# mcogoni/supersdr

Measured on AMD Instinct MI355X. Metric: real-time IQ channels sustained (WF+demod), higher is better.
Workload: dtype f32

## Files before the change

supersdr_amd/csrc/ssdr_audio_dev.h:

```cpp
#pragma once
#include "ssdr_math.h"
#include "ssdr_kernels.h"

constexpr int OCT = 10;
constexpr int NOCT = (SSDR_HIST + SSDR_FRAME) / 8;
constexpr int HOCT = SSDR_HIST / 8;
typedef uint32_t u32x4 __attribute__((ext_vector_type(4)));

SSDR_DEV void lds_sync()
{
    __builtin_amdgcn_fence(__ATOMIC_RELEASE, "wavefront");
    __builtin_amdgcn_wave_barrier();
    __builtin_amdgcn_fence(__ATOMIC_ACQUIRE, "wavefront");
}

template <int CTRL, int ROWMASK>
SSDR_DEV float dpp(float identity, float x)
{
    return __int_as_float(__builtin_amdgcn_update_dpp(__float_as_int(identity), __float_as_int(x), CTRL, ROWMASK, 0xF, false));
}
SSDR_DEV float vmax(float a, float b)
{
    float r;
    asm("v_max_f32 %0, %1, %2" : "=v"(r) : "v"(a), "v"(b));
    return r;
}
SSDR_DEV float vmax3(float a, float b, float c)
{
    float r;
    asm("v_max3_f32 %0, %1, %2, %3" : "=v"(r) : "v"(a), "v"(b), "v"(c));
    return r;
}
SSDR_DEV float vmax3_abs(float a, float b, float c)
{
    float r;
    asm("v_max3_f32 %0, %1, |%2|, |%3|" : "=v"(r) : "v"(a), "v"(b), "v"(c));
    return r;
}
SSDR_DEV uint32_t lane63_u(uint32_t x) { return (uint32_t)__builtin_amdgcn_readlane((int)x, 63); }
SSDR_DEV uint32_t from_prev_lane_u(uint32_t lane0_value, uint32_t x)
{
    return (uint32_t)__builtin_amdgcn_update_dpp((int)lane0_value, (int)x, 0x138, 0xF, 0xF, false);
}
typedef short s16x2 __attribute__((ext_vector_type(2)));
typedef unsigned short u16x2 __attribute__((ext_vector_type(2)));
SSDR_DEV uint32_t iq_power(uint32_t raw)
{
    uint32_t p;
    asm("v_dot2_i32_i16 %0, %1, %1, 0" : "=v"(p) : "v"(raw));
    return p;
}
SSDR_DEV float lane63(float x) { return __int_as_float(__builtin_amdgcn_readlane(__float_as_int(x), 63)); }
SSDR_DEV float from_prev_lane(float lane0_value, float x) { return dpp<0x138, 0xF>(lane0_value, x); }

#define SSDR_SCAN6(STEP) STEP("row_shr:1", "0xf") STEP("row_shr:2", "0xf") STEP("row_shr:4", "0xf") STEP("row_shr:8", "0xf") \
                         STEP("row_bcast:15", "0xa") STEP("row_bcast:31", "0xc")
#define SSDR_DPP(C, M) " " C " row_mask:" M " bank_mask:0xf"

SSDR_DEV float scan_max(float x)
{
#define STEP(C, M) asm("s_nop 1\n\tv_max_f32_dpp %0, %0, %0" SSDR_DPP(C, M) : "+v"(x));
    SSDR_SCAN6(STEP)
#undef STEP
    return x;
}
SSDR_DEV float scan_sum(float x)
{
#define STEP(C, M) asm("s_nop 1\n\tv_add_f32_dpp %0, %0, %0" SSDR_DPP(C, M) : "+v"(x));
    SSDR_SCAN6(STEP)
#undef STEP
    return x;
}
SSDR_DEV void scan_affine(float &A, float &B)
{
#define STEP(C, M) asm("s_nop 1\n\tv_fmac_f32_dpp %1, %1, %0" SSDR_DPP(C, M) "\n\tv_mul_f32_dpp %0, %0, %0" SSDR_DPP(C, M) : "+v"(A), "+v"(B));
    SSDR_SCAN6(STEP)
#undef STEP
}

struct Nco {
    uint32_t dphi;
    float cs, ss;
    float qc, qs;
    float tc, ts;
};
SSDR_DEV void nco_setup(Nco &n, uint32_t dphi, int l, int block = 8)
{
    n.dphi = dphi;
    ssdr_phasor32(dphi, n.cs, n.ss);
    ssdr_phasor32((uint32_t)(block * l) * dphi, n.qc, n.qs);
    n.tc = 1.0f; n.ts = 0.0f;
}
SSDR_DEV void nco_frame_table(Nco &n, uint32_t phase_of_frame, int l, int frame = SSDR_FRAME)
{
    ssdr_phasor32(phase_of_frame + (uint32_t)(frame * l) * n.dphi, n.tc, n.ts);
}
SSDR_DEV float lane_f(float x, uint32_t lane) { return __int_as_float(__builtin_amdgcn_readlane(__float_as_int(x), (int)lane)); }
SSDR_DEV void nco_block(const Nco &n, uint32_t f, float &c, float &s)
{
    const float fc = lane_f(n.tc, f & 63u), fs = lane_f(n.ts, f & 63u);
    c = fmaf(fc, n.qc, -(fs * n.qs));
    s = fmaf(fs, n.qc, fc * n.qs);
}
SSDR_DEV void phasor_mul(float ac, float as, float bc, float bs, float &c, float &s)
{
    c = fmaf(ac, bc, -(as * bs));
    s = fmaf(as, bc, ac * bs);
}

template <bool CLIP, int N = 8>
SSDR_DEV void mix8(const uint32_t (&rw)[N], float c, float s, float cs, float ss, float2 (&z)[N], float &amax)
{
#pragma unroll
    for (int j = 0; j < N; j++) {
        const float xr = (float)(int16_t)(rw[j] & 0xFFFFu);
        const float xi = (float)((int32_t)rw[j] >> 16);
        if (CLIP) amax = vmax3_abs(amax, xr, xi);
        z[j] = make_float2(fmaf(xr, c, xi * s), fmaf(xi, c, -(xr * s)));
        const float cn = fmaf(c, cs, -(s * ss)), sn = fmaf(s, cs, c * ss);
        c = cn; s = sn;
    }
}

template <bool CLIP>
SSDR_DEV void mix8_carry(const uint32_t *rw, float &c, float &s, float cs, float ss, float2 (&z)[8], float &amax)
{
#pragma unroll
    for (int j = 0; j < 8; j++) {
        const float xr = (float)(int16_t)(rw[j] & 0xFFFFu);
        const float xi = (float)((int32_t)rw[j] >> 16);
        if (CLIP) amax = vmax3_abs(amax, xr, xi);
        z[j] = make_float2(fmaf(xr, c, xi * s), fmaf(xi, c, -(xr * s)));
        const float cn = fmaf(c, cs, -(s * ss)), sn = fmaf(s, cs, c * ss);
        c = cn; s = sn;
    }
}

SSDR_DEV void load_oct(const float2 *z, int q, float2 (&v)[8])
{
    const float4 *p = reinterpret_cast<const float4 *>(z + q * OCT);
#pragma unroll
    for (int i = 0; i < 4; i++) {
        const float4 t = p[i];
        v[2 * i] = make_float2(t.x, t.y);
        v[2 * i + 1] = make_float2(t.z, t.w);
    }
}

SSDR_DEV void store_oct(float2 *z, int q, const float2 (&v)[8])
{
    float4 *p = reinterpret_cast<float4 *>(z + q * OCT);
#pragma unroll
    for (int i = 0; i < 4; i++) p[i] = make_float4(v[2 * i].x, v[2 * i].y, v[2 * i + 1].x, v[2 * i + 1].y);
}

template <int K0, int NK>
SSDR_DEV void fir_taps(const float *h, const float2 (&A)[8], const float2 (&B)[8], float (&yr)[8], float (&yi)[8])
{
#pragma unroll
    for (int kk = K0; kk < K0 + NK; kk++) {
#pragma unroll
        for (int j = 0; j < 8; j++) {
            const float2 v = (j - kk >= 0) ? A[(j - kk) & 7] : B[(8 + j - kk) & 7];
            yr[j] = fmaf(h[kk], v.x, yr[j]);
            yi[j] = fmaf(h[kk], v.y, yi[j]);
        }
    }
}


struct AgcK { float c0, c1, knee, d8; uint32_t K; };

template <bool INTEGER_POWER>
SSDR_DEV void demod_am(const float (&p)[8], float &dc, float (&aud)[8])
{
    constexpr float DC_APOW[8] = SSDR_DC_APOW_INIT;
    float env[8], loc[8];
    float s = 0.0f;
#pragma unroll
    for (int j = 0; j < 8; j++) {
        env[j] = INTEGER_POWER ? ssdr_sqrt_rn_int(p[j]) : ssdr_sqrt_rn(p[j]);
        s = fmaf(SSDR_DC_A, s, SSDR_DC_AL * env[j]);
        loc[j] = s;
    }
    float Asc = DC_APOW[7], Bsc = s;
    scan_affine(Asc, Bsc);
    const float Ae = from_prev_lane(1.0f, Asc), Be = from_prev_lane(0.0f, Bsc);
    const float carry = fmaf(Ae, dc, Be);
    float m = 0.0f;
#pragma unroll
    for (int j = 0; j < 8; j++) {
        m = fmaf(DC_APOW[j], carry, loc[j]);
        aud[j] = env[j] - m;
    }
    dc = lane63(m);
}

SSDR_DEV void demod_ssb(const float (&yr)[8], const float (&yi)[8], float c, float s, float cs2, float ss2, float (&aud)[8])
{
#pragma unroll
    for (int j = 0; j < 8; j++) {
        aud[j] = fmaf(yr[j], c, -(yi[j] * s));
        const float cn = fmaf(c, cs2, -(s * ss2)), sn = fmaf(s, cs2, c * ss2);
        c = cn; s = sn;
    }
}

SSDR_DEV void demod_fm(const float (&yr)[8], const float (&yi)[8], float prev_re, float prev_im, float kfm, float (&aud)[8])
{
    float pr = from_prev_lane(prev_re, yr[7]), pi = from_prev_lane(prev_im, yi[7]);
#pragma unroll
    for (int j = 0; j < 8; j++) {
        const float dr = fmaf(yr[j], pr, yi[j] * pi);
        const float di = fmaf(yi[j], pr, -(yr[j] * pi));
        aud[j] = ssdr_atan2p(di, dr) * kfm;
        pr = yr[j]; pi = yi[j];
    }
}

SSDR_DEV float block_peak(const float (&p)[8])
{
    return vmax3(vmax3(vmax3(p[0], p[1], p[2]), p[3], p[4]), vmax3(p[5], p[6], p[7]), SSDR_P_FLOOR);
}

SSDR_DEV float agc_pack_store(const float (&p)[8], const float (&aud)[8], int l, const AgcK &k, float &agc_d,
                              float (&agc_m)[8], int16_t *dst, float pm_known = -1.0f)
{
    const float pm = pm_known >= 0.0f ? pm_known : block_peak(p);
    const float al = ssdr_log2p(pm);
    const float fl = (float)l;
    const float d8 = k.d8;
    float e;
    if (k.K == 0) {
        const float P = scan_max(fmaf(fl, d8, al));
        e = vmax(fmaf(-fl, d8, P), fmaf(-(fl + 1.0f), d8, agc_d));
        agc_d = lane63(e);
    } else {
        const float P = scan_max(al);
        float maxM = agc_m[0], mK = agc_m[0];
#pragma unroll
        for (int i = 1; i < 8; i++)
            if ((uint32_t)i < k.K) { maxM = fmaxf(maxM, agc_m[i]); mK = agc_m[i]; }
        e = vmax(vmax(P, maxM), fmaf(-(fl + 1.0f), d8, agc_d));
        agc_d = fmaxf(fmaf(-64.0f, d8, agc_d), mK);
#pragma unroll
        for (int i = 7; i > 0; i--) agc_m[i] = agc_m[i - 1];
        agc_m[0] = lane63(P);
    }
    const float g = ssdr_exp2p(fmaf(k.c1, vmax(e, k.knee), k.c0));
    u32x4 w;
#pragma unroll
    for (int j = 0; j < 8; j += 2) {
        const int i0 = __float2int_rn(aud[j] * g), i1 = __float2int_rn(aud[j + 1] * g);
        w[j >> 1] = __builtin_bit_cast(uint32_t, __builtin_amdgcn_cvt_pk_i16(i0, i1));
    }
    SSDR_NT_STORE(w, reinterpret_cast<u32x4 *>(dst));
    return g;
}

template <bool HANG> struct AgcHang { float m[8]; };
template <> struct AgcHang<false> {};

template <bool HANG>
SSDR_DEV void agc_pack_store_fused(const float (&aud)[8], int l, const AgcK &k, float &agc_d, AgcHang<HANG> &hang, int16_t *dst, float pm)
{
    const float al = ssdr_log2p(pm);
    const float fl = (float)l;
    const float d8 = k.d8;
    float e;
    auto no_hang = [&] {
        const float P = scan_max(fmaf(fl, d8, al));
        e = vmax(fmaf(-fl, d8, P), fmaf(-(fl + 1.0f), d8, agc_d));
        agc_d = lane63(e);
    };
    if constexpr (!HANG) {
        no_hang();
    } else if (k.K == 0) {
        no_hang();
    } else {
        float (&agc_m)[8] = hang.m;
        const float P = scan_max(al);
        float maxM = agc_m[0], mK = agc_m[0];
#pragma unroll
        for (int i = 1; i < 8; i++)
            if ((uint32_t)i < k.K) { maxM = fmaxf(maxM, agc_m[i]); mK = agc_m[i]; }
        e = vmax(vmax(P, maxM), fmaf(-(fl + 1.0f), d8, agc_d));
        agc_d = fmaxf(fmaf(-64.0f, d8, agc_d), mK);
#pragma unroll
        for (int i = 7; i > 0; i--) agc_m[i] = agc_m[i - 1];
        agc_m[0] = lane63(P);
    }
    const float g = ssdr_exp2p(fmaf(k.c1, vmax(e, k.knee), k.c0));
    u32x4 w;
#pragma unroll
    for (int j = 0; j < 8; j += 2) {
        const int i0 = __float2int_rn(aud[j] * g), i1 = __float2int_rn(aud[j + 1] * g);
        w[j >> 1] = __builtin_bit_cast(uint32_t, __builtin_amdgcn_cvt_pk_i16(i0, i1));
    }
    SSDR_NT_STORE(w, reinterpret_cast<u32x4 *>(dst));
}

SSDR_DEV void iq_pack_store(const float (&yr)[8], const float (&yi)[8], float g, uint32_t *dst)
{
    u32x4 w0, w1;
#pragma unroll
    for (int j = 0; j < 8; j++) {
        const uint32_t v = __builtin_bit_cast(uint32_t, __builtin_amdgcn_cvt_pk_i16(__float2int_rn(yr[j] * g), __float2int_rn(yi[j] * g)));
        if (j < 4) w0[j] = v; else w1[j - 4] = v;
    }
    SSDR_NT_STORE(w0, reinterpret_cast<u32x4 *>(dst));
    SSDR_NT_STORE(w1, reinterpret_cast<u32x4 *>(dst) + 1);
}

SSDR_DEV void rssi_flag_step(const float (&p)[8], bool clip, uint32_t f, uint32_t n_frames, int l, float cal,
                             float &rssi_sum, uint32_t &flag_keep, float *rssi_row, uint8_t *flag_row)
{
    float ps = p[0];
#pragma unroll
    for (int j = 1; j < 8; j++) ps = ps + p[j];
    const float tot = lane63(scan_sum(ps));
    if ((f & 63u) == (uint32_t)l) { rssi_sum = tot; flag_keep = clip ? 1u : 0u; }
    if ((f & 63u) == 63u || f + 1 == n_frames) {
        if ((uint32_t)l <= (f & 63u)) {
            rssi_row[(f & ~63u) + l] = fmaf(ssdr_log2p(fmaxf(rssi_sum, 1e-20f)) - 39.0f, SSDR_DB_PER_LOG2, cal);
            flag_row[(f & ~63u) + l] = (uint8_t)flag_keep;
        }
    }
}

SSDR_DEV bool wave_any(bool x) { return __builtin_amdgcn_ballot_w64(x) != 0ull; }

SSDR_DEV bool raw_clipped(const uint32_t (&rw)[8])
{
    bool c = false;
#pragma unroll
    for (int j = 0; j < 8; j++) {
        const int lo = (int16_t)(rw[j] & 0xFFFFu), hi = (int32_t)rw[j] >> 16;
        c = c || lo >= 32767 || lo <= -32767 || hi >= 32767 || hi <= -32767;
    }
    return c;
}

SSDR_DEV bool raw_clipped1(uint32_t rw)
{
    const int lo = (int16_t)(rw & 0xFFFFu), hi = (int32_t)rw >> 16;
    return lo >= 32767 || lo <= -32767 || hi >= 32767 || hi <= -32767;
}
SSDR_DEV bool raw_clipped_delayed(const uint32_t (&rw)[8], uint32_t last, int l)
{
    bool head = false, c = raw_clipped1(last);
#pragma unroll
    for (int j = 0; j < 4; j++) head |= raw_clipped1(rw[j]);
#pragma unroll
    for (int j = 4; j < 8; j++) c |= raw_clipped1(rw[j]);
    return c | (head & (l != 0));
}

SSDR_DEV uint32_t scan_add_u(uint32_t x)
{
#define STEP(C, M) asm("s_nop 1\n\tv_add_u32_dpp %0, %0, %0" SSDR_DPP(C, M) : "+v"(x));
    SSDR_SCAN6(STEP)
#undef STEP
    return x;
}
SSDR_DEV uint32_t scan_max_u(uint32_t x)
{
#define STEP(C, M) asm("s_nop 1\n\tv_max_u32_dpp %0, %0, %0" SSDR_DPP(C, M) : "+v"(x));
    SSDR_SCAN6(STEP)
#undef STEP
    return x;
}

struct NbRun { uint32_t gate, thresh, s1, s2, left; };

template <int N>
SSDR_DEV uint32_t nb_frame(uint32_t (&rw)[N], int l, NbRun &s, bool &clip)
{
    constexpr uint32_t M = 64u * N;
    constexpr int SHIFT = __builtin_ctz(M);
    const uint32_t lmin = s.s1 < s.s2 ? s.s1 : s.s2;
    const uint64_t t64 = (uint64_t)s.thresh * lmin;
    const uint32_t tc = (t64 == 0 || t64 >= 0xFFFFFFFFull) ? 0xFFFFFFFFu : (uint32_t)t64;
    uint32_t part = 0, trig = 0;
    u16x2 rails = {0xFFFFu, 0xFFFFu};
#pragma unroll
    for (int j = 0; j < N; j++) {
        const uint32_t p = iq_power(rw[j]);
        part += p >> SHIFT;
        trig |= (uint32_t)(p > tc) << j;
        rails = __builtin_elementwise_min(rails, __builtin_bit_cast(u16x2, rw[j]) + (u16x2){32769u, 32769u});
    }
    clip = wave_any(rails.x < 3u || rails.y < 3u);
    const uint32_t n0 = (uint32_t)(N * l);
    const uint32_t le = trig ? n0 + (31u - (uint32_t)__builtin_clz(trig)) + s.gate : 0u;
    const uint32_t sc = scan_max_u(le);
    const uint32_t from_left = from_prev_lane_u(0u, sc);
    const uint32_t e = s.left > from_left ? s.left : from_left;
    int d = (int)e - (int)n0;
    uint32_t mask = 0;
#pragma unroll
    for (int j = 0; j < N; j++) {
        d = (trig >> j) & 1u ? j + (int)s.gate : d;
        const bool b = j < d;
        mask |= (uint32_t)b << j;
        rw[j] = b ? 0u : rw[j];
    }
    const uint32_t sum = lane63_u(scan_add_u(part));
    const uint32_t last = lane63_u(sc);
    const uint32_t ef = s.left > last ? s.left : last;
    s.left = ef > M ? ef - M : 0u;
    s.s2 = s.s1;
    s.s1 = sum;
    return mask;
}
```

supersdr_amd/csrc/ssdr_wf.hip:

```cpp
#include "ssdr_math.h"
#include "ssdr_kernels.h"
#include "ssdr_audio_dev.h"
#include "ssdr_wf_dev.h"

namespace {

constexpr int WAVES = SSDR_WF_BLOCK / 64;
constexpr int LDS_TOTAL = LDS_XCH + WAVES * 2 * XCH_FLOATS * 4;
static_assert(LDS_TOTAL <= 163840, "LDS budget");

template <bool AVG, bool HOP>
__global__ __launch_bounds__(SSDR_WF_BLOCK, SSDR_WF_WAVES_PER_EU) void ssdr_wf_kernel(SsdrWfArgs a)
{
    __shared__ __attribute__((aligned(16))) unsigned char smem[LDS_TOTAL];
    load_tables(smem, a.win, a.tw_stage, a.lut);

    const int lane = threadIdx.x & 63, wave = __builtin_amdgcn_readfirstlane(threadIdx.x >> 6);
    const int h = lane >> 5, l = lane & 31;
    float *xch_wave = reinterpret_cast<float *>(smem + LDS_XCH) + wave * 2 * XCH_FLOATS;
    const unsigned char *lut = smem + LDS_LUT0;
    const uint32_t n_pairs = (a.n_ch + 1) >> 1;
    const uint32_t run = HOP ? a.grp_run : 1u;
    const uint32_t n_runs = (a.n_groups + run - 1) / run;
    const uint32_t n_items = n_pairs * n_runs;
    const uint32_t wave_stride = gridDim.x * WAVES;

    for (uint32_t item = blockIdx.x * WAVES + wave; item < n_items; item += wave_stride) {
      uint32_t pair, g_begin, g_end;
      if (HOP) {
          pair = item / n_runs;
          g_begin = (item - pair * n_runs) * run;
          g_end = min(g_begin + run, a.n_groups);
      } else {
          g_begin = item / n_pairs;
          pair = item - g_begin * n_pairs;
          g_end = g_begin + 1;
      }
      const uint32_t n_trips = HOP ? g_end - g_begin : 1u;
      for (uint32_t trip = 0; trip < n_trips; trip++) {
        const uint32_t grp = g_begin + trip;
        uint32_t pair_now = __builtin_amdgcn_readfirstlane(pair);
        asm volatile("" : "+s"(pair_now));
        const WfItem it = wf_item(a, pair_now, grp, h);
        const float calq = a.consts[it.ch].wf_cal_lin * SSDR_LUT_SCALE;
        uint32_t acc[AVG ? 16 : 1];
#pragma unroll
        for (int j = 0; j < (AVG ? 16 : 1); j++) acc[j] = 0;
        constexpr uint32_t LINE_STEP = HOP ? SSDR_NFFT / 2 : SSDR_NFFT;
        const uint32_t *src = a.iq + (uint64_t)it.ch * a.ch_stride + (uint64_t)it.l0 * LINE_STEP + l;

        for (uint32_t line = it.l0; line < it.l1; line++, src += LINE_STEP) {
            f32x2 z[32];
            uint32_t raw[32];
            if (HOP) load_line_halves(line ? src - SSDR_NFFT / 2 : a.tail + (uint64_t)it.ch * (SSDR_NFFT / 2) + l, src, raw);
            else load_line(src, raw);
            if (SSDR_PRIO_WF) prio_compute_phase();
            window_line(raw, smem, l, z);
            SCHED_FENCE();
            fft_line<AVG>(z, smem, xch_wave, h, l);
            if (SSDR_PRIO_WF) prio_latency_phase();

            if (AVG) {
                quantise32(z, calq, lut, [&](int j, uint32_t q01) { acc[j] += q01; });
            } else {
                uint32_t q[16];
                quantise32(z, calq, lut, [&](int j, uint32_t q01) { q[j] = q01; });
                int16_t *x16 = reinterpret_cast<int16_t *>(xch_wave + opaque(h) * XCH_FLOATS) + opaque(l);
#pragma unroll
                for (int j = 0; j < 16; j++) {
                    x16[32 * (j + 16)] = (int16_t)(q[j] & 0xFFFFu);
                    x16[32 * j] = (int16_t)(q[j] >> 16);
                }
            }
        }

        float *xch = xch_wave + opaque(h) * XCH_FLOATS;
        if (AVG) {
            int16_t *x16 = reinterpret_cast<int16_t *>(xch) + opaque(l);
#pragma unroll
            for (int j = 0; j < 16; j++) {
                x16[32 * (j + 16)] = (int16_t)(acc[j] & 0xFFFFu);
                x16[32 * j] = (int16_t)(acc[j] >> 16);
            }
        }
        wave_lds_sync();
        const u32x4 *x128 = reinterpret_cast<const u32x4 *>(xch);
        int16_t *dst = it.complete ? a.out + ((uint64_t)it.grp * a.n_ch + it.ch) * SSDR_NFFT
                                   : a.acc_out + (uint64_t)it.ch * SSDR_NFFT;
        const int16_t *cin = a.acc_in + (uint64_t)it.ch * SSDR_NFFT;
#pragma unroll
        for (int q = 0; q < 4; q++) {
            u32x4 v = x128[q * 32 + l];
            if (AVG && it.carry_in)
                v += reinterpret_cast<const u32x4 *>(cin)[q * 32 + l];
            if (it.ch_ok) SSDR_NT_STORE(v, reinterpret_cast<u32x4 *>(dst) + q * 32 + l);
        }
        wave_lds_sync();
      }
    }
}

template <bool HOP, bool AVG = false, bool HANG = true>
__global__ __launch_bounds__(SSDR_WF_BLOCK, SSDR_WF_WAVES_PER_EU) void ssdr_fused_am_kernel(SsdrFusedArgs fa)
{
    __shared__ __attribute__((aligned(16))) unsigned char smem[LDS_TOTAL];
    const SsdrWfArgs &a = fa.wf;
    const SsdrAudioArgs &u = fa.au;
    load_tables(smem, a.win, a.tw_stage, a.lut);

    const int lane = threadIdx.x & 63, wave = __builtin_amdgcn_readfirstlane(threadIdx.x >> 6);
    const int h = lane >> 5, l = lane & 31;
    float *xch_wave = reinterpret_cast<float *>(smem + LDS_XCH) + wave * 2 * XCH_FLOATS;
    uint32_t *qbuf = reinterpret_cast<uint32_t *>(xch_wave);
    const unsigned char *lut = smem + LDS_LUT0;
    const uint32_t n_pairs = (a.n_ch + 1) >> 1;
    const uint32_t wave_stride = gridDim.x * WAVES;
    const uint32_t n_frames = u.n_frames;

    for (uint32_t pair = blockIdx.x * WAVES + wave; pair < n_pairs; pair += wave_stride) {
        const uint32_t ch_raw = 2 * pair + h;
        const bool ch_ok = ch_raw < a.n_ch;
        const uint32_t ch = ch_ok ? ch_raw : a.n_ch - 1;
        const float cal_wf = a.consts[ch].wf_cal_lin * SSDR_LUT_SCALE;
        const uint32_t n_sub = (2 * pair + 1 < a.n_ch) ? 2u : 1u;

        float rssi_sum[2] = {0.0f, 0.0f};
        uint32_t flag_keep[2] = {0u, 0u};
        auto pad = [&](int c, int i) -> float & { return xch_wave[c * XCH_FLOATS + 33 * (i + 17) + 32]; };
        constexpr int PAD_TAIL = HANG ? 10 : 2;
        constexpr bool PARKED = !HOP;
        constexpr int PARK = PARKED ? 4 : 0;
        if (lane < 2) {
            const uint32_t cc = min(2 * pair + (uint32_t)lane, a.n_ch - 1);
            const ssdr_chan_state st = u.state[cc];
            pad(lane, 0) = st.dc;
            pad(lane, 1) = st.agc_d;
            if (HANG) {
#pragma unroll
                for (int i = 0; i < 8; i++) pad(lane, 2 + i) = st.agc_m[i];
            }
            const uint4 t = *reinterpret_cast<const uint4 *>(u.hist + (size_t)cc * SSDR_HIST + SSDR_HIST - 4);
            if constexpr (PARKED) {
                pad(lane, PAD_TAIL) = __uint_as_float(t.x); pad(lane, PAD_TAIL + 1) = __uint_as_float(t.y);
                pad(lane, PAD_TAIL + 2) = __uint_as_float(t.z); pad(lane, PAD_TAIL + 3) = __uint_as_float(t.w);
            } else {
                pad(lane, PAD_TAIL) = __uint_as_float(iq_power(t.x)); pad(lane, PAD_TAIL + 1) = __uint_as_float(iq_power(t.y));
                pad(lane, PAD_TAIL + 2) = __uint_as_float(iq_power(t.z)); pad(lane, PAD_TAIL + 3) = __uint_as_float(iq_power(t.w));
            }
        }
        wave_lds_sync();

        const uint32_t *src = a.iq + (uint64_t)ch * a.ch_stride + l;
        uint32_t last_raw31 = 0;
        uint32_t acc[AVG ? 16 : 1];
#pragma unroll
        for (int j = 0; j < (AVG ? 16 : 1); j++) acc[j] = 0;
        constexpr uint32_t LINE_STEP = HOP ? SSDR_NFFT / 2 : SSDR_NFFT;
        constexpr int FRAMES_PER_LINE = HOP ? 1 : 2;
        for (uint32_t line = 0; line < a.n_lines; line++, src += LINE_STEP) {
            float dc[2], agc_d[2];
            AgcHang<HANG> hang[2];
            uint32_t tail_q[2][4];
#pragma unroll
            for (int c = 0; c < 2; c++) {
                dc[c] = pad(c, 0); agc_d[c] = pad(c, 1);
                if constexpr (HANG) {
#pragma unroll
                    for (int i = 0; i < 8; i++) hang[c].m[i] = pad(c, 2 + i);
                }
                if constexpr (!PARKED) {
#pragma unroll
                    for (int i = 0; i < 4; i++) tail_q[c][i] = __float_as_uint(pad(c, PAD_TAIL + i));
                }
            }
            if constexpr (PARKED) {
                u32x4 b[2];
#pragma unroll
                for (int c = 0; c < 2; c++)
#pragma unroll
                    for (int i = 0; i < 4; i++) b[c][i] = __float_as_uint(pad(c, PAD_TAIL + i));
                wave_lds_sync();
                if (lane == 0) {
#pragma unroll
                    for (int c = 0; c < 2; c++) *reinterpret_cast<u32x4 *>(qbuf + c * XCH_FLOATS) = b[c];
                }
            }
            wave_lds_sync();
            const uint32_t lw = opaque(lane);
            uint32_t *q_park = qbuf + PARK + 4 * lw;
            const uint32_t *q_lane = q_park - PARK + 4 * lw, *q_last = qbuf + (lw & 3u);
            {
                u32x4 t[2][4];
#pragma unroll
                for (int c = 0; c < 2; c++) {
                    uint32_t pair_now = __builtin_amdgcn_readfirstlane(pair);
                    asm volatile("" : "+s"(pair_now));
                    const uint32_t cc = min(2 * pair_now + (uint32_t)c, a.n_ch - 1);
                    const uint32_t *row = a.iq + (uint64_t)cc * a.ch_stride + (uint64_t)line * LINE_STEP;
                    if (HOP) {
                        const uint32_t *older = line ? row - SSDR_NFFT / 2 : a.tail + (uint64_t)cc * (SSDR_NFFT / 2);
#pragma unroll
                        for (int i = 0; i < 2; i++) t[c][i] = SSDR_NT_LOAD(reinterpret_cast<const u32x4 *>(older) + 64 * i + lw);
#pragma unroll
                        for (int i = 0; i < 2; i++) t[c][2 + i] = reinterpret_cast<const u32x4 *>(row)[64 * i + lw];
                    } else {
#pragma unroll
                        for (int i = 0; i < 4; i++) t[c][i] = SSDR_NT_LOAD(reinterpret_cast<const u32x4 *>(row) + 64 * i + lw);
                    }
                }
                SCHED_FENCE();
#pragma unroll
                for (int c = 0; c < 2; c++)
#pragma unroll
                    for (int i = 0; i < 4; i++) reinterpret_cast<u32x4 *>(q_park + c * XCH_FLOATS)[64 * i] = t[c][i];
                SCHED_FENCE();
            }
            wave_lds_sync();
            prio_latency_phase();
#pragma unroll
            for (int c = 0; c < 2; c++) {
                if ((uint32_t)c >= n_sub) continue;
                uint32_t pair_now = __builtin_amdgcn_readfirstlane(pair);
                asm volatile("" : "+s"(pair_now));
                const uint32_t cc = 2 * pair_now + c;
                const ssdr_chan_consts &kc = u.consts[cc];
                const AgcK agc_c = {kc.agc_c0, kc.agc_c1, kc.agc_knee, kc.agc_delta8, kc.hang_frames};
                const float cal_c = kc.smeter_cal_db;
#pragma unroll
                for (int f = 0; f < FRAMES_PER_LINE; f++) {
                    const uint32_t frame = HOP ? line : 2 * line + f;
                    const int FBASE = c * XCH_FLOATS + SSDR_FRAME * (HOP ? 1 : f);
                    const u32x4 *qp = reinterpret_cast<const u32x4 *>(q_lane + FBASE);
                    const u32x4 q0 = qp[0], q1 = qp[1];
                    const uint32_t rw[8] = {q0.x, q0.y, q0.z, q0.w, q1.x, q1.y, q1.z, q1.w};
                    uint32_t d[8];
                    float p[8], aud[8];
                    float pmx;
                    bool trig, clip;
                    if constexpr (PARKED) {
                        const uint32_t last = q_last[FBASE + SSDR_FRAME];
#pragma unroll
                        for (int j = 0; j < 8; j++) d[j] = iq_power(rw[j]);
#pragma unroll
                        for (int j = 0; j < 8; j++) p[j] = (float)d[j];
                        pmx = block_peak(p);
                        trig = wave_any((pmx >= 1073676160.0f) | (iq_power(last) >= 0x3FFF0001u));
                        clip = trig ? wave_any(raw_clipped_delayed(rw, last, lane)) : false;
                    } else {
                        uint32_t qv[8];
#pragma unroll
                        for (int j = 0; j < 8; j++) qv[j] = iq_power(rw[j]);
#pragma unroll
                        for (int j = 0; j < 4; j++) { d[j] = from_prev_lane_u(tail_q[c][j], qv[4 + j]); d[4 + j] = qv[j]; }
#pragma unroll
                        for (int j = 0; j < 4; j++) tail_q[c][j] = lane63_u(qv[4 + j]);
#pragma unroll
                        for (int j = 0; j < 8; j++) p[j] = (float)d[j];
                        pmx = block_peak(p);
                        trig = wave_any(pmx >= 1073676160.0f) || tail_q[c][0] >= 0x3FFF0001u || tail_q[c][1] >= 0x3FFF0001u ||
                               tail_q[c][2] >= 0x3FFF0001u || tail_q[c][3] >= 0x3FFF0001u;
                        clip = trig ? wave_any(raw_clipped(rw)) : false;
                    }
                    demod_am<true>(p, dc[c], aud);
                    agc_pack_store_fused<HANG>(aud, lane, agc_c, agc_d[c], hang[c], u.pcm + ((uint64_t)cc * n_frames + frame) * SSDR_FRAME + 8 * lane, pmx);
                    rssi_flag_step(p, clip, frame, n_frames, lane, cal_c, rssi_sum[c], flag_keep[c],
                                   u.rssi + (uint64_t)cc * n_frames, u.flags + (uint64_t)cc * n_frames);
                }
            }
            wave_lds_sync();
            prio_compute_phase();
            uint32_t raw[32];
            {
                const uint32_t *q = qbuf + opaque(h) * XCH_FLOATS + opaque(l);
#pragma unroll
                for (int r = 0; r < 32; r++) raw[r] = q[PARK + 32 * r];
            }
            wave_lds_sync();
            if (lane < 2) {
#pragma unroll
                for (int c = 0; c < 2; c++) {
                    if (lane != c) continue;
                    pad(c, 0) = dc[c]; pad(c, 1) = agc_d[c];
                    if constexpr (HANG) {
#pragma unroll
                        for (int i = 0; i < 8; i++) pad(c, 2 + i) = hang[c].m[i];
                    }
                    if constexpr (PARKED) {
                        const u32x4 e = *reinterpret_cast<const u32x4 *>(qbuf + c * XCH_FLOATS + PARK + SSDR_NFFT - 4);
#pragma unroll
                        for (int i = 0; i < 4; i++) pad(c, PAD_TAIL + i) = __uint_as_float(e[i]);
                    } else {
#pragma unroll
                        for (int i = 0; i < 4; i++) pad(c, PAD_TAIL + i) = __uint_as_float(tail_q[c][i]);
                    }
                }
            }
            wave_lds_sync();
            SCHED_FENCE();
            if (line + 1 == a.n_lines && ch_ok) {
#pragma unroll
                for (int r = 28; r < 32; r++) u.hist[(size_t)ch * SSDR_HIST + 32 * (r - 28) + l] = raw[r];
            }
            last_raw31 = raw[31];
            uint32_t qn[16];
            f32x2 z[32];
            window_line(raw, smem, l, z);
            SCHED_FENCE();
            fft_line<true>(z, smem, xch_wave, h, l);
            prio_latency_phase();
            if (AVG) quantise32(z, cal_wf, lut, [&](int j, uint32_t q01) { acc[j] += q01; });
            else quantise32(z, cal_wf, lut, [&](int j, uint32_t q01) { qn[j] = q01; });
            const uint32_t pos = a.phase + line;
            const bool group_done = !AVG || (pos + 1) % a.n_avg == 0;
            const bool last_line = line + 1 == a.n_lines;
            if (group_done || last_line) {
                float *xch = xch_wave + opaque(h) * XCH_FLOATS;
                int16_t *x16 = reinterpret_cast<int16_t *>(xch) + opaque(l);
#pragma unroll
                for (int j = 0; j < 16; j++) {
                    const uint32_t v = AVG ? acc[j] : qn[j];
                    x16[32 * (j + 16)] = (int16_t)(v & 0xFFFFu);
                    x16[32 * j] = (int16_t)(v >> 16);
                }
                wave_lds_sync();
                const u32x4 *x128 = reinterpret_cast<const u32x4 *>(xch);
                const uint32_t grp = AVG ? pos / a.n_avg : line;
                int16_t *dst = group_done ? a.out + ((uint64_t)grp * a.n_ch + ch) * SSDR_NFFT : a.acc_out + (uint64_t)ch * SSDR_NFFT;
                const bool carry_in = AVG && grp == 0 && a.phase != 0;
                const int16_t *cin = a.acc_in + (uint64_t)ch * SSDR_NFFT;
#pragma unroll
                for (int q = 0; q < 4; q++) {
                    u32x4 v = x128[q * 32 + l];
                    if (carry_in) v += reinterpret_cast<const u32x4 *>(cin)[q * 32 + l];
                    if (ch_ok) SSDR_NT_STORE(v, reinterpret_cast<u32x4 *>(dst) + q * 32 + l);
                }
                wave_lds_sync();
                if (AVG) {
#pragma unroll
                    for (int j = 0; j < 16; j++) acc[j] = 0;
                }
            }
        }

        if (a.n_lines) {
            uint32_t parg = 0;
#pragma unroll
            for (int c = 0; c < 2; c++) {
                if ((uint32_t)c >= n_sub) continue;
                const uint32_t cc = 2 * pair + c;
                const uint32_t dphi1 = u.consts[cc].dphi1;
                const uint32_t phi_last = u.state[cc].phi1 + (uint32_t)(SSDR_FRAME * (n_frames - 1)) * dphi1;
                parg = lane == 3 * c ? phi_last : lane == 3 * c + 1 ? (uint32_t)(8 * 63) * dphi1 : lane == 3 * c + 2 ? dphi1 : parg;
            }
            float pcos, psin;
            ssdr_phasor32(parg, pcos, psin);
#pragma unroll
            for (int c = 0; c < 2; c++) {
                if ((uint32_t)c >= n_sub) continue;
                const uint32_t cc = 2 * pair + c;
                const ssdr_chan_consts &kc = u.consts[cc];
                ssdr_chan_state st = u.state[cc];
                const float fc = lane_f(pcos, 3 * c), fs = lane_f(psin, 3 * c), qc = lane_f(pcos, 3 * c + 1), qs = lane_f(psin, 3 * c + 1);
                const float cs = lane_f(pcos, 3 * c + 2), ss = lane_f(psin, 3 * c + 2);
                float bc, bs;
                phasor_mul(fc, fs, qc, qs, bc, bs);
#pragma unroll
                for (int j = 0; j < 3; j++) { const float cn = fmaf(bc, cs, -(bs * ss)), sn = fmaf(bs, cs, bc * ss); bc = cn; bs = sn; }
                const float xr = (float)(int16_t)(last_raw31 & 0xFFFFu), xi = (float)((int32_t)last_raw31 >> 16);
                const float zr = fmaf(xr, bc, xi * bs) + 0.0f, zi = fmaf(xi, bc, -(xr * bs)) + 0.0f;
                st.prev_re = lane_f(zr, 32 * c + 27);
                st.prev_im = lane_f(zi, 32 * c + 27);
                st.phi1 += (uint32_t)(SSDR_FRAME * n_frames) * kc.dphi1;
                st.phi2 += (uint32_t)(SSDR_FRAME * n_frames) * kc.dphi2;
                st.dc = pad(c, 0); st.agc_d = pad(c, 1);
                if (HANG) {
#pragma unroll
                    for (int i = 0; i < 8; i++) st.agc_m[i] = pad(c, 2 + i);
                }
                if (lane == 0) u.state[cc] = st;
            }
        }
    }
}

__global__ __launch_bounds__(256) void ssdr_quant_selftest_kernel(const float *thr_g, const uint32_t *lut_g,
                                                                    unsigned long long *mismatch)
{
    __shared__ __attribute__((aligned(16))) unsigned char smem[LDS_LUT_END + 16 + 1024];
    float *s_thr = reinterpret_cast<float *>(smem + ((LDS_LUT_END + 15) & ~15));
    uint32_t *s_lut = reinterpret_cast<uint32_t *>(smem + LDS_LUT0);
    for (int i = threadIdx.x; i < 256; i += blockDim.x) s_thr[i] = thr_g[i];
    for (int i = threadIdx.x; i < SSDR_LUT_N; i += blockDim.x) s_lut[i] = lut_g[i];
    __syncthreads();
    unsigned long long bad = 0;
    const unsigned char *lut = smem + LDS_LUT0;
    const uint64_t stride = (uint64_t)gridDim.x * blockDim.x;
    for (uint64_t u = (uint64_t)blockIdx.x * blockDim.x + threadIdx.x; u < 0x7F800000ull; u += stride) {
        const float p = __uint_as_float((uint32_t)u);
        int lo = 0, hi = 255;
        while (lo < hi) {
            const int mid = (lo + hi + 1) >> 1;
            if (s_thr[mid] <= p) lo = mid; else hi = mid - 1;
        }
        float pc;
        asm("v_mul_f32_e64 %0, %1, %2 clamp" : "=v"(pc) : "v"(p), "v"(SSDR_LUT_SCALE));
        bad += (quantise(pc, lut) != (uint32_t)lo);
    }
    if (bad) atomicAdd(mismatch, bad);
}

}

hipError_t ssdr_launch_wf(const SsdrWfArgs &a, uint32_t grid, hipStream_t stream)
{
    const dim3 g(grid), b(SSDR_WF_BLOCK);
    if (a.tail) {
        if (a.n_avg > 1) hipLaunchKernelGGL((ssdr_wf_kernel<true, true>), g, b, 0, stream, a);
        else hipLaunchKernelGGL((ssdr_wf_kernel<false, true>), g, b, 0, stream, a);
    } else {
        if (a.n_avg > 1) hipLaunchKernelGGL((ssdr_wf_kernel<true, false>), g, b, 0, stream, a);
        else hipLaunchKernelGGL((ssdr_wf_kernel<false, false>), g, b, 0, stream, a);
    }
    return hipGetLastError();
}

template <bool HANG>
static void launch_fused_am(const SsdrFusedArgs &a, uint32_t grid, hipStream_t stream)
{
    if (a.wf.n_avg > 1) {
        if (a.wf.tail) hipLaunchKernelGGL((ssdr_fused_am_kernel<true, true, HANG>), dim3(grid), dim3(SSDR_WF_BLOCK), 0, stream, a);
        else hipLaunchKernelGGL((ssdr_fused_am_kernel<false, true, HANG>), dim3(grid), dim3(SSDR_WF_BLOCK), 0, stream, a);
    } else {
        if (a.wf.tail) hipLaunchKernelGGL((ssdr_fused_am_kernel<true, false, HANG>), dim3(grid), dim3(SSDR_WF_BLOCK), 0, stream, a);
        else hipLaunchKernelGGL((ssdr_fused_am_kernel<false, false, HANG>), dim3(grid), dim3(SSDR_WF_BLOCK), 0, stream, a);
    }
}

hipError_t ssdr_launch_fused_am(const SsdrFusedArgs &a, uint32_t grid, hipStream_t stream, bool any_hang)
{
    if (any_hang) launch_fused_am<true>(a, grid, stream);
    else launch_fused_am<false>(a, grid, stream);
    return hipGetLastError();
}

template <bool HANG>
static hipError_t fused_blocks_per_cu(int *blocks)
{
    int b[4] = {0, 0, 0, 0};
    hipError_t e = hipOccupancyMaxActiveBlocksPerMultiprocessor(&b[0], ssdr_fused_am_kernel<false, false, HANG>, SSDR_WF_BLOCK, 0);
    if (e == hipSuccess) e = hipOccupancyMaxActiveBlocksPerMultiprocessor(&b[1], ssdr_fused_am_kernel<true, false, HANG>, SSDR_WF_BLOCK, 0);
    if (e == hipSuccess) e = hipOccupancyMaxActiveBlocksPerMultiprocessor(&b[2], ssdr_fused_am_kernel<false, true, HANG>, SSDR_WF_BLOCK, 0);
    if (e == hipSuccess) e = hipOccupancyMaxActiveBlocksPerMultiprocessor(&b[3], ssdr_fused_am_kernel<true, true, HANG>, SSDR_WF_BLOCK, 0);
    for (int i = 0; i < 4; i++) *blocks = b[i] < *blocks ? b[i] : *blocks;
    return e;
}

hipError_t ssdr_fused_blocks_per_cu(int *blocks)
{
    *blocks = 0x7fffffff;
    hipError_t e = fused_blocks_per_cu<true>(blocks);
    if (e == hipSuccess) e = fused_blocks_per_cu<false>(blocks);
    return e;
}

hipError_t ssdr_wf_blocks_per_cu(int *blocks)
{
    int b[4] = {0, 0, 0, 0};
    hipError_t e = hipOccupancyMaxActiveBlocksPerMultiprocessor(&b[0], ssdr_wf_kernel<false, false>, SSDR_WF_BLOCK, 0);
    if (e == hipSuccess) e = hipOccupancyMaxActiveBlocksPerMultiprocessor(&b[1], ssdr_wf_kernel<true, false>, SSDR_WF_BLOCK, 0);
    if (e == hipSuccess) e = hipOccupancyMaxActiveBlocksPerMultiprocessor(&b[2], ssdr_wf_kernel<false, true>, SSDR_WF_BLOCK, 0);
    if (e == hipSuccess) e = hipOccupancyMaxActiveBlocksPerMultiprocessor(&b[3], ssdr_wf_kernel<true, true>, SSDR_WF_BLOCK, 0);
    if (e != hipSuccess) return e;
    *blocks = b[0];
    for (int i = 1; i < 4; i++) *blocks = b[i] < *blocks ? b[i] : *blocks;
    return hipSuccess;
}

hipError_t ssdr_launch_quant_selftest(const float *thr, const uint32_t *lut, unsigned long long *mismatch, hipStream_t stream)
{
    hipLaunchKernelGGL(ssdr_quant_selftest_kernel, dim3(2048), dim3(256), 0, stream, thr, lut, mismatch);
    return hipGetLastError();
}
```

Measured before the change: 44.66 million.

## Table-driven DC scan, uniform RSSI writelane, SGPR-based PCM stores in fused AM kernel

Replaces the AM demod DC-removal scan with an affine scan whose per-lane multiplier constants are computed once per block and kept in extra LDS, so each frame only runs the additive DPP scan. RSSI and flag bookkeeping now use writelane instead of per-lane compares. PCM stores use inline asm with a scalar frame base plus lane byte offset, and loads use precomputed lane byte offsets. The goal is fewer VALU and DPP ops and less address arithmetic per frame. In exchange it uses more LDS, relies on hand-placed s_nop padding in asm, and tightens the LDS budget so two workgroups must still fit per CU.

```diff
diff --git a/supersdr_amd/csrc/ssdr_audio_dev.h b/supersdr_amd/csrc/ssdr_audio_dev.h
--- a/supersdr_amd/csrc/ssdr_audio_dev.h
+++ b/supersdr_amd/csrc/ssdr_audio_dev.h
@@ -261,8 +261,12 @@
 template <bool HANG> struct AgcHang { float m[8]; };
 template <> struct AgcHang<false> {};
 
+#ifndef SSDR_PCM_STORE_FRONT_PAD
+#define SSDR_PCM_STORE_FRONT_PAD "s_nop 4\n\t"
+#endif
 template <bool HANG>
-SSDR_DEV void agc_pack_store_fused(const float (&aud)[8], int l, const AgcK &k, float &agc_d, AgcHang<HANG> &hang, int16_t *dst, float pm)
+SSDR_DEV void agc_pack_store_fused(const float (&aud)[8], int l, const AgcK &k, float &agc_d, AgcHang<HANG> &hang, int16_t *frame,
+                                   uint32_t lane_bytes, float pm)
 {
     const float al = ssdr_log2p(pm);
     const float fl = (float)l;
@@ -297,7 +301,7 @@
         const int i0 = __float2int_rn(aud[j] * g), i1 = __float2int_rn(aud[j + 1] * g);
         w[j >> 1] = __builtin_bit_cast(uint32_t, __builtin_amdgcn_cvt_pk_i16(i0, i1));
     }
-    SSDR_NT_STORE(w, reinterpret_cast<u32x4 *>(dst));
+    asm volatile(SSDR_PCM_STORE_FRONT_PAD "global_store_dwordx4 %0, %1, %2 nt\n\ts_nop 1" : : "v"(lane_bytes), "v"(w), "s"(frame) : "memory");
 }
 
 SSDR_DEV void iq_pack_store(const float (&yr)[8], const float (&yi)[8], float g, uint32_t *dst)
@@ -329,6 +333,85 @@
 }
 
 SSDR_DEV bool wave_any(bool x) { return __builtin_amdgcn_ballot_w64(x) != 0ull; }
+SSDR_DEV uint32_t wave_count(bool x) { return (uint32_t)__builtin_popcountll(__builtin_amdgcn_ballot_w64(x)); }
+
+struct DcScan { float a[6]; float ae; };
+
+SSDR_DEV void scan_affine_consts(DcScan &t)
+{
+    constexpr float DC_APOW[8] = SSDR_DC_APOW_INIT;
+    float A = DC_APOW[7];
+    float after[6];
+    int k = 0;
+#define STEP(C, M) asm("s_nop 1\n\tv_mul_f32_dpp %0, %0, %0" SSDR_DPP(C, M) : "+v"(A)); after[k++] = A;
+    SSDR_SCAN6(STEP)
+#undef STEP
+    t.a[0] = DC_APOW[7];
+#pragma unroll
+    for (int i = 1; i < 6; i++) t.a[i] = after[i - 1];
+    t.ae = from_prev_lane(1.0f, after[5]);
+}
+SSDR_DEV float from_prev_lane_or_zero(float x)
+{
+    return __int_as_float(__builtin_amdgcn_update_dpp(__float_as_int(x), __float_as_int(x), 0x138, 0xF, 0xF, true));
+}
+SSDR_DEV void scan_affine_b(float &B, const DcScan &t)
+{
+    int k = 0;
+#define STEP(C, M) asm("s_nop 1\n\tv_fmac_f32_dpp %0, %0, %1" SSDR_DPP(C, M) : "+v"(B) : "v"(t.a[k])); k++;
+    SSDR_SCAN6(STEP)
+#undef STEP
+}
+SSDR_DEV void demod_am_tab(const float (&p)[8], float &dc, float (&aud)[8], const DcScan &t)
+{
+    constexpr float DC_APOW[8] = SSDR_DC_APOW_INIT;
+    float env[8], loc[8];
+    env[0] = ssdr_sqrt_rn_int(p[0]);
+    float s = SSDR_DC_AL * env[0];
+    loc[0] = s;
+#pragma unroll
+    for (int j = 1; j < 8; j++) {
+        env[j] = ssdr_sqrt_rn_int(p[j]);
+        s = fmaf(SSDR_DC_A, s, SSDR_DC_AL * env[j]);
+        loc[j] = s;
+    }
+    float Bsc = s;
+    scan_affine_b(Bsc, t);
+    const float Be = from_prev_lane_or_zero(Bsc);
+    const float carry = fmaf(t.ae, dc, Be);
+    float m = 0.0f;
+#pragma unroll
+    for (int j = 0; j < 8; j++) {
+        m = fmaf(DC_APOW[j], carry, loc[j]);
+        aud[j] = env[j] - m;
+    }
+    dc = lane63(m);
+}
+#if defined(__has_builtin) && __has_builtin(__builtin_amdgcn_writelane)
+SSDR_DEV int ssdr_writelane(int value, int lane, int old) { return __builtin_amdgcn_writelane(value, lane, old); }
+#else
+extern "C" __device__ int ssdr_writelane(int value, int lane, int old) __asm("llvm.amdgcn.writelane.i32");
+#endif
+
+SSDR_DEV void rssi_flag_step_uniform(const float (&p)[8], uint32_t clip, uint32_t f, uint32_t n_frames, int l, float cal,
+                                     float &rssi_sum, uint32_t &flag_keep, float *rssi_row, uint8_t *flag_row)
+{
+    float ps = p[0];
+#pragma unroll
+    for (int j = 1; j < 8; j++) ps = ps + p[j];
+    const float tot = lane63(scan_sum(ps));
+    rssi_sum = __int_as_float(ssdr_writelane(__float_as_int(tot), (int)(f & 63u), __float_as_int(rssi_sum)));
+    flag_keep = (uint32_t)ssdr_writelane((int)clip, (int)(f & 63u), (int)flag_keep);
+    if ((f & 63u) == 63u || f + 1 == n_frames) {
+        uint32_t lx = (uint32_t)l;
+        asm volatile("" : "+v"(lx));
+        if (lx <= (f & 63u)) {
+            char *r = reinterpret_cast<char *>(rssi_row + (f & ~63u));
+            *reinterpret_cast<float *>(r + (lx << 2)) = fmaf(ssdr_log2p(fmaxf(rssi_sum, 1e-20f)) - 39.0f, SSDR_DB_PER_LOG2, cal);
+            (flag_row + (f & ~63u))[lx] = (uint8_t)flag_keep;
+        }
+    }
+}
 
 SSDR_DEV bool raw_clipped(const uint32_t (&rw)[8])
 {
diff --git a/supersdr_amd/csrc/ssdr_wf.hip b/supersdr_amd/csrc/ssdr_wf.hip
--- a/supersdr_amd/csrc/ssdr_wf.hip
+++ b/supersdr_amd/csrc/ssdr_wf.hip
@@ -8,6 +8,10 @@
 constexpr int WAVES = SSDR_WF_BLOCK / 64;
 constexpr int LDS_TOTAL = LDS_XCH + WAVES * 2 * XCH_FLOATS * 4;
 static_assert(LDS_TOTAL <= 163840, "LDS budget");
+constexpr int LDS_SCAN = LDS_TOTAL;
+constexpr int LDS_SCAN_BYTES = 6 * 64 * 4;
+constexpr int LDS_TOTAL_FUSED = LDS_SCAN + LDS_SCAN_BYTES;
+static_assert(LDS_SCAN % 4 == 0 && 2 * LDS_TOTAL_FUSED <= 163840, "two workgroups per CU");
 
 template <bool AVG, bool HOP>
 __global__ __launch_bounds__(SSDR_WF_BLOCK, SSDR_WF_WAVES_PER_EU) void ssdr_wf_kernel(SsdrWfArgs a)
@@ -100,12 +104,31 @@
     }
 }
 
+template <typename T>
+SSDR_DEV u32x4 *lane_at(T *base, uint32_t lane_bytes)
+{
+    return reinterpret_cast<u32x4 *>(reinterpret_cast<char *>(base) + lane_bytes);
+}
+template <typename T>
+SSDR_DEV const u32x4 *lane_at(const T *base, uint32_t lane_bytes)
+{
+    return reinterpret_cast<const u32x4 *>(reinterpret_cast<const char *>(base) + lane_bytes);
+}
+
 template <bool HOP, bool AVG = false, bool HANG = true>
 __global__ __launch_bounds__(SSDR_WF_BLOCK, SSDR_WF_WAVES_PER_EU) void ssdr_fused_am_kernel(SsdrFusedArgs fa)
 {
-    __shared__ __attribute__((aligned(16))) unsigned char smem[LDS_TOTAL];
+    __shared__ __attribute__((aligned(16))) unsigned char smem[LDS_TOTAL_FUSED];
     const SsdrWfArgs &a = fa.wf;
     const SsdrAudioArgs &u = fa.au;
+    if (threadIdx.x < 64) {
+        DcScan t;
+        scan_affine_consts(t);
+        float *s_scan = reinterpret_cast<float *>(smem + LDS_SCAN) + threadIdx.x;
+#pragma unroll
+        for (int k = 1; k < 6; k++) s_scan[64 * (k - 1)] = t.a[k];
+        s_scan[64 * 5] = t.ae;
+    }
     load_tables(smem, a.win, a.tw_stage, a.lut);
 
     const int lane = threadIdx.x & 63, wave = __builtin_amdgcn_readfirstlane(threadIdx.x >> 6);
@@ -189,6 +212,7 @@
             const uint32_t lw = opaque(lane);
             uint32_t *q_park = qbuf + PARK + 4 * lw;
             const uint32_t *q_lane = q_park - PARK + 4 * lw, *q_last = qbuf + (lw & 3u);
+            const uint32_t lane16 = lw << 4;
             {
                 u32x4 t[2][4];
 #pragma unroll
@@ -200,12 +224,12 @@
                     if (HOP) {
                         const uint32_t *older = line ? row - SSDR_NFFT / 2 : a.tail + (uint64_t)cc * (SSDR_NFFT / 2);
 #pragma unroll
-                        for (int i = 0; i < 2; i++) t[c][i] = SSDR_NT_LOAD(reinterpret_cast<const u32x4 *>(older) + 64 * i + lw);
-#pragma unroll
-                        for (int i = 0; i < 2; i++) t[c][2 + i] = reinterpret_cast<const u32x4 *>(row)[64 * i + lw];
+                        for (int i = 0; i < 2; i++) t[c][i] = SSDR_NT_LOAD(lane_at(older, lane16) + 64 * i);
+#pragma unroll
+                        for (int i = 0; i < 2; i++) t[c][2 + i] = lane_at(row, lane16)[64 * i];
                     } else {
 #pragma unroll
-                        for (int i = 0; i < 4; i++) t[c][i] = SSDR_NT_LOAD(reinterpret_cast<const u32x4 *>(row) + 64 * i + lw);
+                        for (int i = 0; i < 4; i++) t[c][i] = SSDR_NT_LOAD(lane_at(row, lane16) + 64 * i);
                     }
                 }
                 SCHED_FENCE();
@@ -216,6 +240,18 @@
                 SCHED_FENCE();
             }
             wave_lds_sync();
+            DcScan dcs;
+            {
+                constexpr float DC_APOW[8] = SSDR_DC_APOW_INIT;
+                uint32_t scan_base = LDS_SCAN;
+                asm volatile("" : "+s"(scan_base));
+                const float *s_scan = reinterpret_cast<const float *>(smem + scan_base) + lw;
+                dcs.a[0] = DC_APOW[7];
+                asm volatile("" : "+v"(dcs.a[0]));
+#pragma unroll
+                for (int k = 1; k < 6; k++) dcs.a[k] = s_scan[64 * (k - 1)];
+                dcs.ae = s_scan[64 * 5];
+            }
             prio_latency_phase();
 #pragma unroll
             for (int c = 0; c < 2; c++) {
@@ -236,7 +272,8 @@
                     uint32_t d[8];
                     float p[8], aud[8];
                     float pmx;
-                    bool trig, clip;
+                    bool trig;
+                    uint32_t clip;
                     if constexpr (PARKED) {
                         const uint32_t last = q_last[FBASE + SSDR_FRAME];
 #pragma unroll
@@ -245,7 +282,7 @@
                         for (int j = 0; j < 8; j++) p[j] = (float)d[j];
                         pmx = block_peak(p);
                         trig = wave_any((pmx >= 1073676160.0f) | (iq_power(last) >= 0x3FFF0001u));
-                        clip = trig ? wave_any(raw_clipped_delayed(rw, last, lane)) : false;
+                        clip = trig ? (wave_count(raw_clipped_delayed(rw, last, lane)) + 63u) >> 6 : 0u;
                     } else {
                         uint32_t qv[8];
 #pragma unroll
@@ -259,12 +296,12 @@
                         pmx = block_peak(p);
                         trig = wave_any(pmx >= 1073676160.0f) || tail_q[c][0] >= 0x3FFF0001u || tail_q[c][1] >= 0x3FFF0001u ||
                                tail_q[c][2] >= 0x3FFF0001u || tail_q[c][3] >= 0x3FFF0001u;
-                        clip = trig ? wave_any(raw_clipped(rw)) : false;
+                        clip = trig ? (wave_count(raw_clipped(rw)) + 63u) >> 6 : 0u;
                     }
-                    demod_am<true>(p, dc[c], aud);
-                    agc_pack_store_fused<HANG>(aud, lane, agc_c, agc_d[c], hang[c], u.pcm + ((uint64_t)cc * n_frames + frame) * SSDR_FRAME + 8 * lane, pmx);
-                    rssi_flag_step(p, clip, frame, n_frames, lane, cal_c, rssi_sum[c], flag_keep[c],
-                                   u.rssi + (uint64_t)cc * n_frames, u.flags + (uint64_t)cc * n_frames);
+                    demod_am_tab(p, dc[c], aud, dcs);
+                    agc_pack_store_fused<HANG>(aud, lane, agc_c, agc_d[c], hang[c], u.pcm + ((uint64_t)cc * n_frames + frame) * SSDR_FRAME, lane16, pmx);
+                    rssi_flag_step_uniform(p, clip, frame, n_frames, lane, cal_c, rssi_sum[c], flag_keep[c],
+                                           u.rssi + (uint64_t)cc * n_frames, u.flags + (uint64_t)cc * n_frames);
                 }
             }
             wave_lds_sync();
```

After: 45.35 million (median of 6 runs). 1.02x the previous value.
